# kunpengcompute/media

Measured on AMD Instinct MI355X. Metric: encoded fps @1080p I420 baseline-profile, 1/2/4/8 MI355X vs OpenH264 CPU, higher is better.
Workload: dtype u8

## Files before the change

### media_amd/csrc/engine.h

```cpp
#pragma once

#define HIPCHK(err, call)                                                                                    \
    do {                                                                                                     \
        hipError_t _r = (call);                                                                              \
        if (_r != hipSuccess) return set_err((err), MI355X_H264_E_HIP, "%s: %s", #call, hipGetErrorString(_r)); \
    } while (0)
namespace { thread_local const char* t_failed_call = ""; }
#define HIPTRY(call)                                                      \
    do {                                                                  \
        hipError_t _r = (call);                                           \
        if (_r != hipSuccess) { t_failed_call = #call; return _r; }       \
    } while (0)

namespace {

struct DevMem {
    struct Block { void* p; bool pinned; };
    std::vector<Block> blocks;
    template <class T> hipError_t dev(T** p, size_t bytes, bool zero = false)
    {
        HIPTRY(hipMalloc((void**)p, bytes));
        blocks.push_back({*p, false});
        if (zero) HIPTRY(hipMemset(*p, 0, bytes));
        return hipSuccess;
// ... 276 lines not shown
    }
    P.itemtab = T.d_itemtab; P.srctab = T.d_srctab; P.qtab = e->d_qtab; P.st_ring_y = e->st_ring_y; P.st_ring_c = e->st_ring_c; P.nbuf = e->nbuf;
    P.st_src = T.src_item_stride; P.sl = e->sl;
    P.band.row0 = e->b_row0; P.band.rows = e->b_rows;
    const unsigned pic_serial = P.pic_serial;
    const unsigned G = (unsigned)T.n;
    fill_qp(P.qy, P.qc, P.lambda, P.sad_nz, e->qp);
    P.search = e->cfg.search;
    const StepSync& Y = *T.sync;
    hipStream_t st = Y.st;


    if (T.inj) {
        const size_t n = (size_t)T.n * e->nmb;
        HIPCHK(e->err, hipMemcpyAsync(e->d_mb, T.inj->mbinfo, n * sizeof(MbInfo), hipMemcpyHostToDevice, st));
        HIPCHK(e->err, hipMemcpyAsync(e->d_levels, T.inj->levels, n * LV_STRIDE * sizeof(int16_t), hipMemcpyHostToDevice, st));
        HIPCHK(e->err, hipMemcpyAsync(e->d_mvq, T.inj->mvq, n * 8 * sizeof(int16_t), hipMemcpyHostToDevice, st));
        HIPCHK(e->err, hipMemcpyAsync(e->d_aux, T.inj->mbaux, n * 16, hipMemcpyHostToDevice, st));
        HIPCHK(e->err, hipMemsetAsync(e->d_me_cost, 0, n * sizeof(uint16_t), st));
        unsigned anypcm[MAX_BATCH] = {}, anyintra[MAX_BATCH] = {};
        const MbInfo* m = (const MbInfo*)T.inj->mbinfo;
        for (int g = 0; g < T.n; g++)
            for (int i = 0; i < e->nmb; i++) {
                const int type = m[(size_t)g * e->nmb + i].type;
                if (type == MB_IPCM) anypcm[g] = pic_serial;
                if (!idr && mb_is_intra_host(type)) anyintra[g] = pic_serial;
            }
        HIPCHK(e->err, hipMemcpyAsync(e->d_anypcm, anypcm, (size_t)T.n * sizeof(unsigned), hipMemcpyHostToDevice, st));
        HIPCHK(e->err, hipMemcpyAsync(e->d_anyintra, anyintra, (size_t)T.n * sizeof(unsigned), hipMemcpyHostToDevice, st));
        HIPCHK(e->err, hipStreamSynchronize(st));
    } else if (idr) {
        StatScope sc(e, &S, MI355X_H264_K_INTRA, (uint32_t)(e->diag_mode ? e->mbw + e->mbh - 1 : 1), (uint32_t)(e->b_nmb * T.n), st);
        LAUNCH2(ind, k_i4_decide<true>, k_i4_decide<false>, dim3((e->b_nmb + 3) / 4, G), dim3(64), st, P, 0);
        if (e->diag_mode && !ind) {
            for (int s = 0; s < e->mbw + e->mbh - 1; s++) {
                const int ymin = std::max(0, s - e->mbw + 1), ymax = std::min(e->mbh - 1, s);
                hipLaunchKernelGGL(k_intra_diag, dim3(ymax - ymin + 1, G), dim3(64), 0, st, P, s);
            }
        } else {
            const IntraRowParams R = intra_row_params(e, P, Y.h_err, (int)G);
            {
                static const int slots = getenv("MI355X_H264_INTRA_SLOTS") ? std::max(1, atoi(getenv("MI355X_H264_INTRA_SLOTS"))) : 24;
                LAUNCH2(ind, k_intra_rows<true>, k_intra_rows<false>, dim3(e->b_rows, std::min(G, (unsigned)slots)), dim3(128), st, R);
            }
        }
    } else {
        { const bool turns = g_turns_on && !ind && e->me_turn > 0 && T.n >= TURN_MIN_BATCH;
          if (turns) hipLaunchKernelGGL(k_turn_acquire, dim3(1), dim3(64), 0, st, g_turns.d_lock[e->device], (unsigned)e->me_turn, (int)TURN_TIMEOUT_US);
          { StatScope sc(e, &S, MI355X_H264_K_ME, (uint32_t)P.nref, (uint32_t)(e->b_nmb * T.n), st);
            FrameParams Q = P;
            Q.rf_last = P.nref - 1;
            for (int r = 0; r < P.nref; r++) {
                Q.rf = r;
                for (int p = 0; p < 3; p++) Q.ref[p] = P.refs[r][p];
                LAUNCH2(ind, k_me<true>, k_me<false>, dim3(e->b_nmb, G), dim3(64), st, Q);
            } }
          if (turns) hipLaunchKernelGGL(k_turn_release, dim3(1), dim3(1), 0, st, g_turns.d_lock[e->device], (unsigned)e->me_turn);
        }
        { StatScope sc(e, &S, MI355X_H264_K_PMB, 1, (uint32_t)(e->b_nmb * T.n), st);
          if (e->cfg.profile_idc == 100) LAUNCH2(ind, k_tq8<true>, k_tq8<false>, dim3((e->b_nmb + 15) / 16, G), dim3(64), st, P);
          else LAUNCH2(ind, k_tq<true>, k_tq<false>, dim3((e->b_nmb + 7) / 8, G), dim3(64), st, P); }
        {
            const IntraRowParams R = intra_row_params(e, P, Y.h_err, (int)G);
            static const int pslots_env = getenv("MI355X_H264_PINTRA_SLOTS") ? std::max(1, atoi(getenv("MI355X_H264_PINTRA_SLOTS"))) : 0;
            const unsigned pslots = std::min(G, pslots_env ? (unsigned)pslots_env : (e->p_intra_x16 > 16u * PINTRA_SPARSE_MBS ? G : 1u));
            LAUNCH2(ind, k_i4_decide<true>, k_i4_decide<false>, dim3(std::min((e->b_nmb + 3) / 4, (int)I4_MARKED_WAVES), pslots), dim3(64), st, P, (int)G);
            LAUNCH2(ind, (k_pintra_rows<false, true>), (k_pintra_rows<false, false>), dim3(e->b_rows, pslots), dim3(64), st, R);
        }
    }
    HdrBatch H{}, Hpcm{};
    for (int g = 0; g < T.n; g++) {
        uint64_t hdr = 0;
        const int fn = ind ? T.items[g].frame_num : e->seq.frame_num, qp = ind ? T.items[g].qp : e->qp;
        const int id = ind ? T.items[g].idr_id : ((e->seq.idr_id + g * e->idr_step) & 0xFF);
        const int nact = ind ? (idr ? 0 : 1) : avail_refs(e, idr);
        H.len[g] = (unsigned char)build_slice_header(e->shape, idr, id, false, fn, qp, nact, &hdr);
        H.bits[g] = hdr;
        Hpcm.len[g] = (unsigned char)build_slice_header(e->shape, idr, id, true, fn, qp, nact, &hdr);
        Hpcm.bits[g] = hdr;
    }
    hipStream_t ec = T.one_stream ? st : Y.ec;
    CavlcParams C{};
    C.mb = e->d_mb; C.levels = e->d_levels; C.mvd = e->d_mvd; C.mbw = e->mbw; C.nmb = e->nmb; C.p_slice = idr ? 0 : 1; C.t8x8 = e->cfg.profile_idc == 100 ? 1 : 0;
    C.nref = ind ? (idr ? 0 : 1) : avail_refs(e, idr); C.sl = e->sl;
    C.mb_first = e->b_row0 * e->mbw; C.mb_end = C.mb_first + e->b_nmb;
    C.slice_cap = (unsigned)e->slice_cap;
    C.mbdiv = P.mbdiv;
    C.slotbits = e->d_slotbits; C.slotcode = e->d_slotcode; C.mbbits = e->d_mbbits; C.bitbuf = S.d_bitbuf;
    C.bs = (uint8_t*)e->d_bs; C.prevcoded = e->d_prevcoded;
    C.st_mb = e->nmb; C.st_bitbuf = e->st_bitbuf_bytes / 4;
    C.aux = e->d_aux; C.mvq = e->d_mvq;
    C.src = T.d_src; C.w = e->cfg.width; C.h = e->cfg.height; C.src_nv12 = T.nv12 ? 1 : 0; C.st_src = T.src_item_stride;
    C.itemtab = T.d_itemtab; C.srctab = T.d_srctab;
    const int cavlc_grid = (e->b_nmb + 1) / 2;
    unsigned db_serial = 0;
    if (!e->cfg.disable_deblock) {
        db_serial = next_nonzero(e->serial);
        LAUNCH2(ind, k_bs<true>, k_bs<false>, dim3(std::min(cavlc_grid, (int)BS_WAVES), G), dim3(64), st, C, e->d_anybs, db_serial);
    }
    const bool fork = ec != st;
    if (fork) {
        HIPCHK(e->err, hipEventRecord(Y.recon_ready, st));
        HIPCHK(e->err, hipStreamWaitEvent(ec, Y.recon_ready, 0));
    }
    {
        StatScope sc(e, &S, MI355X_H264_K_CAVLC, 4, (uint32_t)(e->b_nmb * T.n), ec);
        const int grid = cavlc_grid;
        if (!idr) {
            LAUNCH2(ind, k_mvpred<true>, k_mvpred<false>, dim3((e->b_nmb + 63) / 64, G), dim3(64), ec, P);
            LAUNCH2(ind, k_skip_scan<true>, k_skip_scan<false>, dim3(G), dim3(256), ec, C);
        }
        LAUNCH2(ind, (k_cavlc<false, true>), (k_cavlc<false, false>), dim3(grid, G), dim3(64), ec, C);
        LAUNCH2(ind, k_bit_scan<true>, k_bit_scan<false>, dim3(G * (unsigned)e->b_nsl), dim3(SCAN_NT), ec, C, H, Hpcm, (const unsigned*)e->d_anypcm, pic_serial, S.d_info, e->d_me_cost,
                e->b_nsl, e->b_sl0, (unsigned)e->slice_cap);
        LAUNCH2(ind, (k_cavlc<true, true>), (k_cavlc<true, false>), dim3(grid, G), dim3(64), ec, C);
        const size_t pre = (idr ? e->sps_pps.size() : 0) + 5;
        const size_t pad = (16 - (pre & 15)) & 15;
        T.lay = AuLayout{pad, e->nsl > 1 ? 0 : pad + pre, idr, idr ? ((3 << 5) | 5) : ((2 << 5) | 1)};
        LAUNCH2(ind, k_pack<true>, k_pack<false>, dim3(G * (unsigned)e->b_nsl), dim3(SCAN_NT), ec, (uint8_t*)S.d_bitbuf, e->st_bitbuf_bytes, S.h_au + T.lay.payload_off, e->st_au,
                (const SliceInfo*)S.d_info, S.h_info, e->b_nsl, e->b_sl0, (unsigned)e->slice_cap, T.d_itemtab);
    }
    if (fork) HIPCHK(e->err, hipEventRecord(Y.entropy_done, ec));
    if (e->keep_pre && !ind && !T.inj)
        for (int p = 0; p < 3; p++) {
            const size_t ring = p ? e->st_ring_c : e->st_ring_y;
            HIPCHK(e->err, hipMemcpy2DAsync(e->d_pre[p], ring, e->d_planes[cur][p], p ? e->st_c : e->st_y, ring, (size_t)e->G, hipMemcpyDeviceToDevice, st));
        }
    if (e->keep_pre && ind)
        for (int k = 0; k < T.n; k++)
            for (int p = 0; p < 3; p++) {
                const size_t ring = p ? e->st_ring_c : e->st_ring_y;
                HIPCHK(e->err, hipMemcpyAsync(e->d_pre[p] + (size_t)T.items[k].item * ring,
                                              e->d_plane_base[p] + (size_t)T.items[k].item * (p ? e->st_c : e->st_y) + (size_t)T.items[k].cur * ring, ring,
                                              hipMemcpyDeviceToDevice, st));
            }
    if (!e->cfg.disable_deblock && !T.inj) {
        const int steps = e->mbw + 2 * (e->mbh - 1);
        StatScope sc(e, &S, MI355X_H264_K_DEBLOCK, (uint32_t)(e->diag_mode ? steps : 1), (uint32_t)(e->b_nmb * T.n), st);
        const DbParams D = db_params(e, ind ? e->d_plane_base : e->d_planes[cur], e->sl, e->qp);
        if (e->diag_mode && !ind) {
            for (int s = 0; s < steps; s++) {
                const int ymin = std::max(0, (s - (e->mbw - 1) + 1) >> 1), ymax = std::min(e->mbh - 1, s >> 1);
                if (ymax < ymin) continue;
                hipLaunchKernelGGL(k_deblock_diag, dim3(ymax - ymin + 1), dim3(64), 0, st, D, s);
            }
        } else {
            DbRowParams R = db_row_params(e, D, Y.h_err, db_serial, pic_serial, e->b_row0, (int)G);
            R.itemtab = T.d_itemtab; R.st_ring_y = e->st_ring_y; R.st_ring_c = e->st_ring_c;
            const bool pairs = e->pair_filter && T.n >= e->pair_min_batch && e->nsl == 1 && e->b_rows == e->mbh;
            const unsigned grid_x = pairs ? (unsigned)((e->b_rows + 1) / 2) : (unsigned)e->b_rows;
            auto filter = [&](bool bs4, unsigned at_a_time) {
                const dim3 grid(grid_x, std::min(G, at_a_time));
                if (pairs) { if (bs4) LAUNCH2(ind, (k_deblock_pairs<true, true>), (k_deblock_pairs<true, false>), grid, dim3(64), st, R);
                             else LAUNCH2(ind, (k_deblock_pairs<false, true>), (k_deblock_pairs<false, false>), grid, dim3(64), st, R); }
                else { if (bs4) LAUNCH2(ind, (k_deblock_rows<true, false, true>), (k_deblock_rows<true, false, false>), grid, dim3(64), st, R);
                       else LAUNCH2(ind, (k_deblock_rows<false, false, true>), (k_deblock_rows<false, false, false>), grid, dim3(64), st, R); }
            };
            if (idr) { R.need_intra = 0; filter(true, G); }
            else {
                R.need_intra = -1; filter(false, G);
                R.need_intra = 1; filter(true, e->p_intra_x16 > 16u * PINTRA_SPARSE_MBS ? G : 1u);
            }
        }
    }
    if (fork) HIPCHK(e->err, hipStreamWaitEvent(st, Y.entropy_done, 0));
    HIPCHK(e->err, hipEventRecord(Y.done, st));
    HIPCHK(e->err, hipGetLastError());
    return MI355X_H264_OK;
}

int submit(mi355x_h264_encoder* e, const uint8_t* d_src, size_t src_item_stride, int slot_idx, bool nv12, const Injected* inj = nullptr)
{
    Slot& S = e->slots[slot_idx];
    const bool idr = e->seq.next_is_idr(e->cfg.gop) || (e->after_injected && !inj);
    e->seq.begin(idr);
    e->after_injected = inj != nullptr;
    Step T;
    T.d_src = d_src; T.src_item_stride = src_item_stride; T.nv12 = nv12; T.idr = idr; T.n = e->G;
    T.sync = &S.sync;
    T.slot = &S;
    T.inj = inj;
    const int rc = submit_step(e, T);
    if (rc) return rc;
    S.lay = T.lay;
    S.busy = true;
    e->seq.advance(idr, e->nbuf, e->idr_step * e->G);
    return MI355X_H264_OK;
}

int wait_slot(mi355x_h264_encoder* e, int slot_idx)
{
    Slot& S = e->slots[slot_idx];
    if (!S.busy) return set_err(e->err, MI355X_H264_E_INTERNAL, "collect on an idle slot");
    HIPCHK(e->err, hipEventSynchronize(S.sync.done));
    S.busy = false;
    for (auto& ev : S.evs) {
        float ms = 0;
        if (hipEventElapsedTime(&ms, ev.a, ev.b) == hipSuccess) {
            e->stats.ms[ev.k] += ms; e->stats.launches[ev.k] += ev.launches; e->stats.mbs[ev.k] += ev.mbs;
        }
        e->ev_pool.push_back(ev.a); e->ev_pool.push_back(ev.b);
    }
    S.evs.clear();
    e->stats.frames += (uint64_t)e->G;
    const int rc = handoff_timeout(S.sync, e->err);
    if (rc) e->seq.force_idr = 1;
    return rc;
}

int finish_item(mi355x_h264_encoder* e, Slot& S, const AuLayout& L, int g, uint8_t** out, uint32_t* out_len, int* frame_type)
{
    uint8_t* base = S.h_au + (size_t)g * e->st_au;
    const SliceInfo* const info = S.h_info + (size_t)g * e->b_nsl;
    for (int sl = 0; sl < e->b_nsl; sl++)
        if (info[sl].error) {
            e->seq.force_idr = 1;
            const int code = info[sl].error == 1 ? MI355X_H264_E_OVERFLOW : MI355X_H264_E_INTERNAL;
            if (e->nsl > 1) return set_err(e->err, code, "device reported error %u (slice %d)", info[sl].error, sl);
            return set_err(e->err, code, "device reported error %u", info[sl].error);
        }
    uint32_t cost = 0, searched = 0, tq_coded = 0;
    size_t need = e->sps_pps.size() + 16;
    for (int sl = 0; sl < e->b_nsl; sl++) {
        cost += info[sl].me_cost; searched += info[sl].searched; tq_coded += info[sl].tq_coded;
        need += 5 + (size_t)info[sl].total_bytes * 3 / 2 + 16;
    }
    e->last_me_cost[g] = cost;
    if (!L.idr) {
        e->stats.p_mbs += (uint64_t)e->b_nmb; e->stats.me_searched_mbs += searched; e->stats.tq_coded_mbs += tq_coded;
        e->p_intra_x16 = (3 * e->p_intra_x16 + 16 * (searched - tq_coded)) / 4;
    }
    if (frame_type) *frame_type = L.idr ? MI355X_H264_FRAME_IDR : MI355X_H264_FRAME_P;
    std::vector<uint8_t>& eb = e->esc_buf[g];
    if (e->nsl > 1) {
        eb.resize(need);
        size_t pos = 0;
        if (L.idr && e->b_sl0 == 0) { memcpy(eb.data(), e->sps_pps.data(), e->sps_pps.size()); pos = e->sps_pps.size(); }
        for (int sl = 0; sl < e->b_nsl; sl++) {
            const SliceInfo& si = info[sl];
            const uint8_t* pay = base + (size_t)(e->b_sl0 + sl) * e->slice_cap;
            uint8_t* o = eb.data() + pos;
            o[0] = 0; o[1] = 0; o[2] = 0; o[3] = 1; o[4] = (uint8_t)L.nal_hdr;
            pos += 5;
            if (si.epb_count == 0) { memcpy(eb.data() + pos, pay, si.total_bytes); pos += si.total_bytes; }
            else pos += nal_escape(pay, si.total_bytes, eb.data() + pos);
        }
        *out = eb.data();
        *out_len = (uint32_t)pos;
        return MI355X_H264_OK;
    }
    uint8_t* au = base + L.au_start;
    size_t pos = 0;
    if (L.idr) { memcpy(au, e->sps_pps.data(), e->sps_pps.size()); pos = e->sps_pps.size(); }
    au[pos++] = 0; au[pos++] = 0; au[pos++] = 0; au[pos++] = 1; au[pos++] = (uint8_t)L.nal_hdr;
    if (info->epb_count == 0) {
        *out = au;
        *out_len = (uint32_t)(pos + info->total_bytes);
    } else {
        eb.resize(pos + (size_t)info->total_bytes * 3 / 2 + 16);
        memcpy(eb.data(), au, pos);
        const size_t n = nal_escape(base + L.payload_off, info->total_bytes, eb.data() + pos);
        *out = eb.data();
        *out_len = (uint32_t)(pos + n);
    }
    return MI355X_H264_OK;
}

int collect(mi355x_h264_encoder* e, int slot_idx, uint8_t** out, uint32_t* out_len, int* frame_type)
{
    const int rc = wait_slot(e, slot_idx);
    return rc ? rc : finish_item(e, e->slots[slot_idx], e->slots[slot_idx].lay, 0, out, out_len, frame_type);
}

void destroy_engine(mi355x_h264_encoder* e)
{
    if (!e) return;
    (void)hipSetDevice(e->device);
    if (e->stream) (void)hipStreamSynchronize(e->stream);
    if (e->stream_ec && e->stream_ec != e->stream) (void)hipStreamSynchronize(e->stream_ec);
    e->mem.free_all();
    for (auto& S : e->slots) {
        sync_destroy(S.sync);
        for (auto& ev : S.evs) { (void)hipEventDestroy(ev.a); (void)hipEventDestroy(ev.b); }
    }
    for (auto ev : e->ev_pool) (void)hipEventDestroy(ev);
    if (e->stream_ec && e->stream_ec != e->stream) (void)hipStreamDestroy(e->stream_ec);
    if (e->counted_live) e->counted_live->fetch_sub(1);
    if (e->stream) (void)hipStreamDestroy(e->stream);
    delete e;
}

hipError_t engine_alloc(mi355x_h264_encoder* e, bool hub_engine)
{
    DevMem& M = e->mem;
    HIPTRY(hipSetDevice(e->device));
    HIPTRY(hipStreamCreateWithFlags(&e->stream, hipStreamNonBlocking));
    {
        static std::atomic<int> live{0};
        const char* one = getenv("MI355X_H264_ONE_STREAM");
        const int n = live.fetch_add(1) + 1;
        e->counted_live = &live;
        if ((one && one[0] == '1') || (n > 2 && !(one && one[0] == '0'))) e->stream_ec = e->stream;
        else HIPTRY(hipStreamCreateWithFlags(&e->stream_ec, hipStreamNonBlocking));
    }
    const size_t ysz = (size_t)e->cw * e->ch;
    const size_t Gn = (size_t)e->G, nmb = Gn * e->nmb;
    e->st_ring_y = ysz + 256; e->st_ring_c = ysz / 4 + 256;
    e->st_y = e->st_ring_y * e->nbuf; e->st_c = e->st_ring_c * e->nbuf;
    for (int p = 0; p < 3; p++) {
        HIPTRY(M.dev(&e->d_plane_base[p], (p ? e->st_c : e->st_y) * Gn, true));
        for (int b = 0; b < e->nbuf; b++) e->d_planes[b][p] = e->d_plane_base[p] + (size_t)b * (p ? e->st_ring_c : e->st_ring_y);
    }
// ... 203 lines not shown
```

### media_amd/csrc/k_deblock.h

```cpp
#pragma once
#include "dev_common.h"

namespace h264 {

__constant__ const uint8_t c_alpha[52] = {0,  0,  0,  0,  0,  0,  0,  0,  0,  0,  0,  0,  0,   0,   0,   0,   4,   4,
                                          5,  6,  7,  8,  9,  10, 12, 13, 15, 17, 20, 22, 25,  28,  32,  36,  40,  45,
                                          50, 56, 63, 71, 80, 90, 101, 113, 127, 144, 162, 182, 203, 226, 255, 255};
__constant__ const uint8_t c_beta[52] = {0,  0,  0,  0,  0,  0,  0,  0,  0,  0,  0,  0,  0,  0,  0,  0,  2,  2,
                                         2,  3,  3,  3,  3,  4,  4,  4,  6,  6,  7,  7,  8,  8,  9,  9,  10, 10,
                                         11, 11, 12, 12, 13, 13, 14, 14, 15, 15, 16, 16, 17, 17, 18, 18};
__constant__ const uint8_t c_tc0[52][3] = {
    {0, 0, 0},   {0, 0, 0},   {0, 0, 0},    {0, 0, 0},    {0, 0, 0},    {0, 0, 0},   {0, 0, 0},   {0, 0, 0},  {0, 0, 0},
    {0, 0, 0},   {0, 0, 0},   {0, 0, 0},    {0, 0, 0},    {0, 0, 0},    {0, 0, 0},   {0, 0, 0},   {0, 0, 0},  {0, 0, 1},
    {0, 0, 1},   {0, 0, 1},   {0, 0, 1},    {0, 1, 1},    {0, 1, 1},    {1, 1, 1},   {1, 1, 1},   {1, 1, 1},  {1, 1, 1},
    {1, 1, 2},   {1, 1, 2},   {1, 1, 2},    {1, 1, 2},    {1, 2, 3},    {1, 2, 3},   {2, 2, 3},   {2, 2, 4},  {2, 3, 4},
    {2, 3, 4},   {3, 3, 5},   {3, 4, 6},    {3, 4, 6},    {4, 5, 7},    {4, 5, 8},   {4, 6, 9},   {5, 7, 10}, {6, 8, 11},
    {6, 8, 13},  {7, 10, 14}, {8, 11, 16},  {9, 12, 18},  {10, 13, 20}, {11, 15, 23}, {13, 17, 25}};

struct DbParams {
    uint8_t* pl[3];
    const MbInfo* mb;
    int cw, ch, mbw, mbh;
    int alpha_y, beta_y, alpha_c, beta_c;
    int tc0_y[3], tc0_c[3];
// ... 24 lines not shown
    const int ap = iabs(p2 - p0), aq = iabs(q2 - q0);
    if (bS < 4) {
        const int tc = tc0 + (ap < beta) + (aq < beta);
        const int d = clip3(-tc, tc, (((q0 - p0) << 2) + (p1 - q1) + 4) >> 3);
        pix[-xs] = (uint8_t)clip255(p0 + d);
        pix[0] = (uint8_t)clip255(q0 - d);
        if (ap < beta) pix[-2 * xs] = (uint8_t)(p1 + clip3(-tc0, tc0, (p2 + ((p0 + q0 + 1) >> 1) - (p1 << 1)) >> 1));
        if (aq < beta) pix[xs] = (uint8_t)(q1 + clip3(-tc0, tc0, (q2 + ((p0 + q0 + 1) >> 1) - (q1 << 1)) >> 1));
    } else {
        const int p3 = pix[-4 * xs], q3 = pix[3 * xs];
        const bool strong = iabs(p0 - q0) < ((alpha >> 2) + 2);
        if (ap < beta && strong) {
            pix[-xs] = (uint8_t)((p2 + 2 * p1 + 2 * p0 + 2 * q0 + q1 + 4) >> 3);
            pix[-2 * xs] = (uint8_t)((p2 + p1 + p0 + q0 + 2) >> 2);
            pix[-3 * xs] = (uint8_t)((2 * p3 + 3 * p2 + p1 + p0 + q0 + 4) >> 3);
        } else pix[-xs] = (uint8_t)((2 * p1 + p0 + q1 + 2) >> 2);
        if (aq < beta && strong) {
            pix[0] = (uint8_t)((p1 + 2 * p0 + 2 * q0 + 2 * q1 + q2 + 4) >> 3);
            pix[xs] = (uint8_t)((p0 + q0 + q1 + q2 + 2) >> 2);
            pix[2 * xs] = (uint8_t)((2 * q3 + 3 * q2 + q1 + q0 + p0 + 4) >> 3);
        } else pix[0] = (uint8_t)((2 * q1 + q0 + p1 + 2) >> 2);
    }
}

enum { DB_LP = 24, DB_CP = 12 };

__global__ __launch_bounds__(64) void k_deblock_diag(DbParams D, int s)
{
    const int lane = threadIdx.x;
    const int ymin = max(0, (s - (D.mbw - 1) + 1) >> 1);
    const int my = ymin + blockIdx.x, mx = s - 2 * my;
    if (my >= D.mbh || mx < 0 || mx >= D.mbw) return;
    const int cs = D.cw / 2;
    __shared__ __attribute__((aligned(16))) uint8_t s_y[20 * DB_LP];
    __shared__ __attribute__((aligned(16))) uint8_t s_c[2][10 * DB_CP];
    __shared__ uint8_t s_bs[2][16];

    for (int i = lane; i < 20 * 5; i += 64) {
        const int r = i / 5, c = i - r * 5;
        const int gy = 16 * my - 4 + r, gx = 16 * mx - 4 + c * 4;
        uint32_t v = 0;
        if (gy >= 0 && gx >= 0) v = *(const uint32_t*)(D.pl[0] + (size_t)gy * D.cw + gx);
        *(uint32_t*)(s_y + r * DB_LP + c * 4) = v;
    }
    for (int i = lane; i < 2 * 10 * 5; i += 64) {
        const int pl = i / 50, k = i - pl * 50, r = k / 5, c = k - r * 5;
        const int gy = 8 * my - 2 + r, gx = 8 * mx - 2 + c * 2;
        uint16_t v = 0;
        if (gy >= 0 && gx >= 0) v = *(const uint16_t*)(D.pl[1 + pl] + (size_t)gy * cs + gx);
        *(uint16_t*)(s_c[pl] + r * DB_CP + c * 2) = v;
    }
    if (lane < 32) {
        const int dir = lane >> 4, e = (lane >> 2) & 3, k = lane & 3;
        const int bS = D.bs[((size_t)my * D.mbw + mx) * 32 + lane];
        s_bs[dir][e * 4 + k] = (uint8_t)bS;
    }
    __syncthreads();

    const bool isY = lane < 16, isC = lane >= 16 && lane < 32;
    const int cpl = (lane >> 3) & 1, cl = lane & 7;
#pragma unroll 1
    for (int dir = 0; dir < 2; dir++) {
#pragma unroll 1
        for (int e = 0; e < 4; e++) {
            if (isY) {
                const int bS = s_bs[dir][e * 4 + (lane >> 2)];
                if (bS) {
                    uint8_t* p = dir == 0 ? s_y + (4 + lane) * DB_LP + 4 + 4 * e : s_y + (4 + 4 * e) * DB_LP + 4 + lane;
                    filter_line(p, dir == 0 ? 1 : DB_LP, bS, D.alpha_y, D.beta_y, bS < 4 ? D.tc0_y[bS - 1] : 0, false);
                }
            } else if (isC && !(e & 1)) {
                const int bS = s_bs[dir][e * 4 + (cl >> 1)];
                if (bS) {
                    uint8_t* p = dir == 0 ? s_c[cpl] + (2 + cl) * DB_CP + 2 + 2 * e : s_c[cpl] + (2 + 2 * e) * DB_CP + 2 + cl;
                    filter_line(p, dir == 0 ? 1 : DB_CP, bS, D.alpha_c, D.beta_c, bS < 4 ? D.tc0_c[bS - 1] : 0, true);
                }
            }
            __syncthreads();
        }
    }
    for (int i = lane; i < 20 * 5; i += 64) {
        const int r = i / 5, c = i - r * 5;
        const int gy = 16 * my - 4 + r, gx = 16 * mx - 4 + c * 4;
        if (gy < 0 || gx < 0) continue;
        if (r < 4 && c == 0) continue;
        *(uint32_t*)(D.pl[0] + (size_t)gy * D.cw + gx) = *(const uint32_t*)(s_y + r * DB_LP + c * 4);
    }
    for (int i = lane; i < 2 * 10 * 5; i += 64) {
        const int pl = i / 50, k = i - pl * 50, r = k / 5, c = k - r * 5;
        const int gy = 8 * my - 2 + r, gx = 8 * mx - 2 + c * 2;
        if (gy < 0 || gx < 0) continue;
        if (r < 2 && c == 0) continue;
        *(uint16_t*)(D.pl[1 + pl] + (size_t)gy * cs + gx) = *(const uint16_t*)(s_c[pl] + r * DB_CP + c * 2);
    }
}

typedef unsigned long long u64;
#define AT_LOAD(p) __hip_atomic_load((p), __ATOMIC_RELAXED, __HIP_MEMORY_SCOPE_AGENT)
#define AT_STORE(p, v) __hip_atomic_store((p), (v), __ATOMIC_RELAXED, __HIP_MEMORY_SCOPE_AGENT)

struct DbRowParams {
    DbParams d;
    u64* handoff;
    const uint32_t* bs;
    unsigned* err;
    unsigned serial;
    const unsigned* anybs;
    const unsigned* anypcm;
    const unsigned* anyintra;
    unsigned pic_serial;
    int npic;
    int need_intra;
    size_t st_y, st_c, st_handoff;
    int st_mb;
    int row0;
    const uint32_t* itemtab;
    size_t st_ring_y, st_ring_c;
    const DecPos* dectab;
};

template <bool BS4>
__device__ __forceinline__ void filt_uni(const int p3, int& p2, int& p1, int& p0, int& q0, int& q1, int& q2, const int q3,
                                         int bS, bool chroma, int alpha, int beta, int t1, int t2, int t3)
{
    const int tc0 = bS == 1 ? t1 : (bS == 2 ? t2 : t3);
    const int fm = -(int)(bS != 0 && iabs(p0 - q0) < alpha && iabs(p1 - p0) < beta && iabs(q1 - q0) < beta);
    const int lum = chroma ? 0 : -1;
    const int apm = lum & -(int)(iabs(p2 - p0) < beta), aqm = lum & -(int)(iabs(q2 - q0) < beta);
    const int tc = tc0 + (chroma ? 1 : 0) - apm - aqm;
    const int d = clip3(-tc, tc, (((q0 - p0) << 2) + (p1 - q1) + 4) >> 3);
    const int avg = (p0 + q0 + 1) >> 1;
    int dp0 = clip255(p0 + d) - p0, dq0 = clip255(q0 - d) - q0;
    int dp1 = apm & clip3(-tc0, tc0, (p2 + avg - (p1 << 1)) >> 1);
    int dq1 = aqm & clip3(-tc0, tc0, (q2 + avg - (q1 << 1)) >> 1);
    int dp2 = 0, dq2 = 0;
    if (BS4) {
        const int s4 = -(int)(bS == 4);
        const int strong = -(int)(iabs(p0 - q0) < ((alpha >> 2) + 2));
        const int sp = apm & strong, sq = aqm & strong;
        const int wp0 = (sp & (((p2 + 2 * p1 + 2 * p0 + 2 * q0 + q1 + 4) >> 3) - p0)) | (~sp & (((2 * p1 + p0 + q1 + 2) >> 2) - p0));
        const int wq0 = (sq & (((p1 + 2 * p0 + 2 * q0 + 2 * q1 + q2 + 4) >> 3) - q0)) | (~sq & (((2 * q1 + q0 + p1 + 2) >> 2) - q0));
        const int wp1 = sp & (((p2 + p1 + p0 + q0 + 2) >> 2) - p1), wq1 = sq & (((p0 + q0 + q1 + q2 + 2) >> 2) - q1);
        const int wp2 = sp & (((2 * p3 + 3 * p2 + p1 + p0 + q0 + 4) >> 3) - p2), wq2 = sq & (((2 * q3 + 3 * q2 + q1 + q0 + p0 + 4) >> 3) - q2);
        dp0 = (s4 & wp0) | (~s4 & dp0); dq0 = (s4 & wq0) | (~s4 & dq0);
        dp1 = (s4 & wp1) | (~s4 & dp1); dq1 = (s4 & wq1) | (~s4 & dq1);
        dp2 = s4 & wp2; dq2 = s4 & wq2;
    }
    p0 += fm & dp0; q0 += fm & dq0; p1 += fm & dp1; q1 += fm & dq1;
    if (BS4) { p2 += fm & dp2; q2 += fm & dq2; }
}

enum { DR_LP = 40, DR_CP = 24 };
enum { DR_CB = 4 * 201, DR_CPS = 4 * 144, DR_TILE = DR_CB + 2 * DR_CPS + 12 };
__device__ __forceinline__ uint8_t* db_y(uint8_t* const tile, const int r, const int c) { return tile + (r + 4) * DR_LP + c + 16; }
__device__ __forceinline__ uint8_t* db_c(uint8_t* const tile, const int pl, const int r, const int c) { return tile + DR_CB + pl * DR_CPS + (r + 4) * DR_CP + c + 8; }
__device__ __forceinline__ uint32_t& dw(uint8_t* const p) { return *(uint32_t*)p; }

struct DbThr { int al, be, t1, t2, t3; };
__device__ __forceinline__ DbThr db_picture_thr(const DbParams& D, const bool isC)
{
    return isC ? DbThr{D.alpha_c, D.beta_c, D.tc0_c[0], D.tc0_c[1], D.tc0_c[2]} : DbThr{D.alpha_y, D.beta_y, D.tc0_y[0], D.tc0_y[1], D.tc0_y[2]};
}
template <bool PERMB, bool IND>
__device__ __forceinline__ bool db_picture_view(const DbRowParams& R, const int pos, DbParams& D, u64*& handoff, const uint32_t*& bsw)
{
    if constexpr (PERMB) {
        const DecPosRef dp = dec_pos(R.dectab, pos);
        if (!dp.filtered || R.anybs[dp.item] != R.serial) return false;
        if (R.need_intra != 0 && dp.intra != (R.need_intra > 0)) return false;
        D = R.d;
        const size_t g = (size_t)dp.item;
        D.pl[0] += g * R.st_y + (size_t)dp.cur * R.st_ring_y; D.pl[1] += g * R.st_c + (size_t)dp.cur * R.st_ring_c; D.pl[2] += g * R.st_c + (size_t)dp.cur * R.st_ring_c;
        D.mb += g * R.st_mb; D.mbqp += g * R.st_mb;
        D.oa = dp.oa; D.ob = dp.ob; D.cqo_cb = dp.cqo_cb; D.cqo_cr = dp.cqo_cr; D.sl = dp.fsl;
        handoff = R.handoff + g * R.st_handoff;
        bsw = R.bs + g * R.st_mb * 8;
        return true;
    } else {
    const int bitem = batch_item<IND>(R.itemtab, pos);
    if (R.anybs[bitem] != R.serial) return false;
    if (R.anypcm[bitem] == R.pic_serial) return false;
    if (R.need_intra != 0 && (R.anyintra[bitem] == R.pic_serial) != (R.need_intra > 0)) return false;
    D = R.d;
    const size_t g = (size_t)bitem;
    D.pl[0] += g * R.st_y; D.pl[1] += g * R.st_c; D.pl[2] += g * R.st_c; D.mb += g * R.st_mb;
    if constexpr (IND) {
        const ItemRef it = item_ref(R.itemtab, pos);
        D.pl[0] += (size_t)it.cur * R.st_ring_y; D.pl[1] += (size_t)it.cur * R.st_ring_c; D.pl[2] += (size_t)it.cur * R.st_ring_c;
        const int qpc = c_chroma_qp[it.qp];
        D.alpha_y = c_alpha[it.qp]; D.beta_y = c_beta[it.qp]; D.alpha_c = c_alpha[qpc]; D.beta_c = c_beta[qpc];
#pragma unroll
        for (int i = 0; i < 3; i++) { D.tc0_y[i] = c_tc0[it.qp][i]; D.tc0_c[i] = c_tc0[qpc][i]; }
    }
    handoff = R.handoff + g * R.st_handoff;
    bsw = R.bs + g * R.st_mb * 8;
    return true;
    }
}
struct DbLane { bool isC; int fpl, seg8, hstride; uint8_t *vrow, *hcol; };
__device__ __forceinline__ DbLane db_lane(const int l, uint8_t* const tile)
{
    DbLane L;
    L.isC = l >= 16; L.fpl = (l >> 3) & 1;
    const int fln = L.isC ? (l & 7) : l;
    L.seg8 = 8 * (L.isC ? (fln >> 1) : (fln >> 2));
    L.vrow = L.isC ? db_c(tile, L.fpl, fln, -4) : db_y(tile, fln, -4);
    L.hcol = L.isC ? db_c(tile, L.fpl, -4, fln) : db_y(tile, -4, fln);
    L.hstride = L.isC ? DR_CP : DR_LP;
    return L;
}
template <bool BS4, int E>
__device__ __forceinline__ bool db_edge(const DbLane& L, int (&px)[20], const uint4 b, const DbThr& T)
{
    const uint32_t w = E == 0 ? b.x : E == 1 ? (L.isC ? b.z : b.y) : E == 2 ? b.z : b.w;
    const int bS = (E >= 2 && L.isC) ? 0 : (int)((w >> L.seg8) & 255);
    if (__ballot(bS != 0) == 0ull) return false;
    filt_uni<BS4>(px[4 * E], px[4 * E + 1], px[4 * E + 2], px[4 * E + 3], px[4 * E + 4], px[4 * E + 5], px[4 * E + 6], px[4 * E + 7],
                  bS, L.isC, T.al, T.be, T.t1, T.t2, T.t3);
    return true;
}
template <int W>
__device__ __forceinline__ uint32_t db_pack(const int (&px)[20])
{
    return (uint32_t)px[4 * W] | ((uint32_t)px[4 * W + 1] << 8) | ((uint32_t)px[4 * W + 2] << 16) | ((uint32_t)px[4 * W + 3] << 24);
}
template <bool BS4>
__device__ __forceinline__ void db_left_edge(const DbLane& L, int (&px)[20], const uint4 b0, const bool on, const DbThr& T)
{
    if (on) {
#pragma unroll
        for (int w = 0; w < 5; w++) {
            const uint32_t v = dw(L.vrow + 4 * w);
#pragma unroll
            for (int b = 0; b < 4; b++) px[4 * w + b] = (int)((v >> (8 * b)) & 255);
        }
        if (db_edge<BS4, 0>(L, px, b0, T)) dw(L.vrow) = db_pack<0>(px);
    }
}
template <bool BS4>
__device__ __forceinline__ void db_inner_vertical(const DbLane& L, int (&px)[20], const uint4 b0, const bool on, const DbThr& T)
{
    if (on) {
        db_edge<BS4, 1>(L, px, b0, T);
        db_edge<BS4, 2>(L, px, b0, T);
        db_edge<BS4, 3>(L, px, b0, T);
        dw(L.vrow + 4) = db_pack<1>(px); dw(L.vrow + 8) = db_pack<2>(px);
        if (!L.isC) { dw(L.vrow + 12) = db_pack<3>(px); dw(L.vrow + 16) = db_pack<4>(px); }
    }
}
template <bool BS4>
__device__ __forceinline__ void db_horizontal(const DbLane& L, const uint4 b1, const bool on, const DbThr& Ttop, const DbThr& T)
{
    if (on) {
        int px[20];
#pragma unroll
        for (int r = 0; r < 20; r++) px[r] = L.hcol[r * L.hstride];
        db_edge<BS4, 0>(L, px, b1, Ttop);
        db_edge<BS4, 1>(L, px, b1, T);
        db_edge<BS4, 2>(L, px, b1, T);
        db_edge<BS4, 3>(L, px, b1, T);
#pragma unroll
        for (int r = 1; r < 19; r++) {
            const bool both = r == 3 || r == 4 || r == 7 || r == 8;
            if (both || !L.isC) L.hcol[r * L.hstride] = (uint8_t)px[r];
        }
    }
}
template <class F>
__device__ __forceinline__ void db_granule(const int k, F f)
{
    if (k < 16) f(false, 0, 12 + (k >> 2), (k & 3) * 4);
    else if (k < 24) f(true, (k - 16) >> 2, 6 + (((k - 16) >> 1) & 1), ((k - 16) & 1) * 4);
}
__device__ __forceinline__ uint8_t* db_tile_at(uint8_t* const tile, const bool c, const int pl, const int r, const int col, const int dmx, const int dmy)
{
    return c ? db_c(tile, pl, 8 * dmy + r, 8 * dmx + col) : db_y(tile, 16 * dmy + r, 16 * dmx + col);
}
__device__ __forceinline__ uint32_t db_bottom_dword(uint8_t* const tile, const int k, const bool shifted)
{
    uint32_t v = 0;
    db_granule(k, [&](bool c, int pl, int r, int col) { v = dw(db_tile_at(tile, c, pl, r, col, shifted ? -1 : 0, 0)); });
    return v;
}
__device__ __forceinline__ void db_put_apron(uint8_t* const tile, const int k, const uint32_t v)
{
    db_granule(k, [&](bool c, int pl, int r, int col) { dw(db_tile_at(tile, c, pl, r, col, 0, -1)) = v; });
}
__device__ __forceinline__ void db_store_apron(const DbParams& D, uint8_t* const tile, const int k, const int mx, const int my)
{
    db_granule(k, [&](bool c, int pl, int r, int col) {
        uint8_t* const p = c ? (pl ? D.pl[2] : D.pl[1]) + (size_t)(8 * (my - 1) + r) * (D.cw / 2) + 8 * mx + col
                             : D.pl[0] + (size_t)(16 * (my - 1) + r) * D.cw + 16 * mx + col;
        dw(p) = dw(db_tile_at(tile, c, pl, r, col, 0, -1));
    });
}
__device__ __forceinline__ void db_wait_tags(const bool need, u64& g, const u64* const addr, const unsigned serial, bool& timed_out)
{
    unsigned spins = 0;
    while (!timed_out) {
        const bool bad = need && (unsigned)(g >> 32) != serial;
        if (__ballot(bad) == 0ull) break;
        if (++spins > (1u << 20)) { timed_out = true; break; }
        __builtin_amdgcn_s_sleep(1);
        if (need) g = AT_LOAD(addr);
    }
}

template <bool BS4, bool PERMB, bool IND>
__device__ __forceinline__ void deblock_rows_picture(const DbRowParams& R, const int pos)
{
    DbParams D; u64* handoff; const uint32_t* bsw;
    if (!db_picture_view<PERMB, IND>(R, pos, D, handoff, bsw)) return;
    const int lane = threadIdx.x, my = R.row0 + blockIdx.x, cs = D.cw / 2;
    const bool first_row = !D.sl.has_top(my);
    const bool last_row = my == D.mbh - 1 || !D.sl.has_top(my + 1);
    __shared__ __attribute__((aligned(16))) uint8_t s_y[DR_TILE];
    bool timed_out = false;
    const int yr = lane >> 2, yc4 = (lane & 3) * 4;
    const int cpl_l = (lane >> 4) & 1, cr_l = (lane >> 1) & 7, cc4 = (lane & 1) * 4;
    const DbLane L = db_lane(lane, s_y);
    DbThr thr = db_picture_thr(D, L.isC), thrL = thr, thrT = thr;
    __shared__ uint32_t s_tA[PERMB ? 52 : 1];
    __shared__ uint8_t s_tB[PERMB ? 52 : 1], s_cq[PERMB ? 52 : 1];
    if (PERMB) {
        if (lane < 52) {
            s_tA[lane] = ((uint32_t)c_alpha[lane] << 24) | ((uint32_t)c_tc0[lane][2] << 16) | ((uint32_t)c_tc0[lane][1] << 8) | (uint32_t)c_tc0[lane][0];
            s_tB[lane] = c_beta[lane];
            s_cq[lane] = c_chroma_qp[lane];
        }
        wave_sync();
    }
    const int cqo = L.fpl ? D.cqo_cr : D.cqo_cb;
    auto thresholds = [&](const int qa, const int qb) {
        const int ca = (int)s_cq[clip3(0, 51, qa + cqo)], cb = (int)s_cq[clip3(0, 51, qb + cqo)];
        const int av = ((L.isC ? ca : qa) + (L.isC ? cb : qb) + 1) >> 1;
        const uint32_t w = s_tA[clip3(0, 51, av + D.oa)];
        return DbThr{(int)(w >> 24), (int)s_tB[clip3(0, 51, av + D.ob)], (int)(w & 255u), (int)((w >> 8) & 255u), (int)((w >> 16) & 255u)};
    };
    uint32_t pf_q = 0;
    int qp_left = 0;

    uint32_t pf_y = 0, pf_c = 0;
    uint4 pf_b0 = {0, 0, 0, 0}, pf_b1 = pf_b0;
    u64 pf_g = 0;
    const int grow = first_row ? my : my - 1;
    const int glane = lane < 24 ? lane : lane - 24 < 24 ? lane - 24 : lane - 48;
    auto prefetch = [&](int mx) {
        pf_y = *(const uint32_t*)(D.pl[0] + (size_t)(16 * my + yr) * D.cw + 16 * mx + yc4);
        pf_c = *(const uint32_t*)((cpl_l ? D.pl[2] : D.pl[1]) + (size_t)(8 * my + cr_l) * cs + 8 * mx + cc4);
        const uint4* b = (const uint4*)(bsw + ((size_t)my * D.mbw + mx) * 8);
        pf_b0 = b[0]; pf_b1 = b[1];
        pf_g = AT_LOAD(handoff + ((size_t)grow * D.mbw + mx) * 24 + glane);
        if (PERMB) pf_q = (uint32_t)D.mbqp[(size_t)my * D.mbw + mx] | ((uint32_t)D.mbqp[(size_t)grow * D.mbw + mx] << 8);
    };
    auto consume = [&]() {
        asm volatile("" : "+v"(pf_y), "+v"(pf_c), "+v"(pf_g));
        asm volatile("" : "+v"(pf_b0.x), "+v"(pf_b0.y), "+v"(pf_b0.z), "+v"(pf_b0.w));
        asm volatile("" : "+v"(pf_b1.x), "+v"(pf_b1.y), "+v"(pf_b1.z), "+v"(pf_b1.w));
        if (PERMB) asm volatile("" : "+v"(pf_q));
    };
    prefetch(0);
    consume();
    uint32_t cur_y = pf_y, cur_c = pf_c, cur_q = pf_q;
    uint4 b0 = pf_b0, b1 = pf_b1;
    u64 g = pf_g;

    auto store_prev = [&](const int mx, const bool have_cur) {
        if (mx > 0) {
            const int pmx = mx - 1;
            const int co = have_cur ? -16 : 0, cco = have_cur ? -8 : 0;
            const int nrow = last_row ? 16 : 12, ncrow = last_row ? 8 : 6;
            if (yr < nrow) *(uint32_t*)(D.pl[0] + (size_t)(16 * my + yr) * D.cw + 16 * pmx + yc4) = dw(db_y(s_y, yr, co + yc4));
            if (lane < 32 && cr_l < ncrow)
                *(uint32_t*)((cpl_l ? D.pl[2] : D.pl[1]) + (size_t)(8 * my + cr_l) * cs + 8 * pmx + cc4) = dw(db_c(s_y, cpl_l, cr_l, cco + cc4));
            if (!last_row && lane < 24)
                AT_STORE(handoff + ((size_t)my * D.mbw + pmx) * 24 + lane, ((u64)R.serial << 32) | db_bottom_dword(s_y, lane, have_cur));
        }
    };
    for (int mx = 0; mx <= D.mbw; mx++) {
        const bool have_cur = mx < D.mbw;
        if (have_cur) {
            if (mx > 0) {
                dw(db_y(s_y, yr, yc4 - 16)) = dw(db_y(s_y, yr, yc4));
                if (lane < 32) dw(db_c(s_y, cpl_l, cr_l, cc4 - 8)) = dw(db_c(s_y, cpl_l, cr_l, cc4));
            }
            wave_sync();
            dw(db_y(s_y, yr, yc4)) = cur_y;
            if (lane < 32) dw(db_c(s_y, cpl_l, cr_l, cc4)) = cur_c;
            if (mx + 1 < D.mbw) prefetch(mx + 1);
            if (PERMB) {
                const int qc = (int)(cur_q & 255u), qt = (int)(cur_q >> 8);
                thr = thresholds(qc, qc);
                thrL = thresholds(mx > 0 ? qp_left : qc, qc);
                thrT = thresholds(qt, qc);
                qp_left = qc;
            }
            wave_sync();
            const bool v_on = (b0.x | b0.y | b0.z | b0.w) != 0 && lane < 32, h_on = (b1.x | b1.y | b1.z | b1.w) != 0 && lane < 32;
            int px[20];
            db_left_edge<BS4>(L, px, b0, v_on, thrL);
            wave_sync();
            store_prev(mx, true);
            db_inner_vertical<BS4>(L, px, b0, v_on, thr);
            if (!first_row) {
                db_wait_tags(lane < 24, g, handoff + ((size_t)grow * D.mbw + mx) * 24 + glane, R.serial, timed_out);
                db_put_apron(s_y, lane, (uint32_t)g);
            }
            wave_sync();
            db_horizontal<BS4>(L, b1, h_on, thrT, thr);
            wave_sync();
            consume();
            if (!first_row) db_store_apron(D, s_y, lane, mx, my);
        }
        if (!have_cur) store_prev(mx, false);
        cur_y = pf_y; cur_c = pf_c; b0 = pf_b0; b1 = pf_b1; g = pf_g; cur_q = pf_q;
        wave_sync();
    }
    if (timed_out && lane == 0) *R.err = 1u;
}
template <bool BS4, bool PERMB = false, bool IND = false>
__global__ __launch_bounds__(64) void k_deblock_rows(DbRowParams R)
{
    static_assert(!PERMB || IND, "thresholds per edge: the pictures of a decoder group's step");
    __builtin_amdgcn_s_setprio(3);
    for (int pos = blockIdx.y; pos < R.npic; pos += gridDim.y) deblock_rows_picture<BS4, PERMB, IND>(R, pos);
}


template <bool BS4, bool IND>
__device__ __forceinline__ void deblock_pairs_picture(const DbRowParams& R, const int pos)
{
    DbParams D; u64* handoff; const uint32_t* bsw;
    if (!db_picture_view<false, IND>(R, pos, D, handoff, bsw)) return;
    const int lane = threadIdx.x, half = lane >> 5, hl = lane & 31, cs = D.cw / 2;
    const int rowA = R.row0 + 2 * (int)blockIdx.x, rowB = rowA + 1;
    const bool hasB = rowB < D.mbh;
    const int my = half ? (hasB ? rowB : rowA) : rowA;
    const bool live = half == 0 || hasB;
    const bool first_row = half == 0 && rowA == 0;
    const bool last_row = my == D.mbh - 1;
    const bool from_lds = half == 1;
    __shared__ __attribute__((aligned(16))) uint8_t s_yy[2][(DR_TILE + 127) / 128 * 128];
    __shared__ __attribute__((aligned(16))) uint32_t s_ring[2][24];
    uint8_t* const s_y = s_yy[half];
    bool timed_out = false;
    const int yr0 = hl >> 2, yc4 = (hl & 3) * 4;
    const int cpl_l = (hl >> 4) & 1, cr_l = (hl >> 1) & 7, cc4 = (hl & 1) * 4;
    const DbLane L = db_lane(hl, s_y);
    const DbThr thr = db_picture_thr(D, L.isC);

    uint32_t pf_y0 = 0, pf_y1 = 0, pf_c = 0;
    uint4 pf_b0 = {0, 0, 0, 0}, pf_b1 = pf_b0;
    u64 pf_g = 0;
    const int grow = (first_row || half == 1) ? rowA : rowA - 1;
    const int glane = hl < 24 ? hl : hl - 24;
    const int last_mx = D.mbw - 1;
    auto prefetch = [&](int mx) {
        pf_y0 = *(const uint32_t*)(D.pl[0] + (size_t)(16 * my + yr0) * D.cw + 16 * mx + yc4);
        pf_y1 = *(const uint32_t*)(D.pl[0] + (size_t)(16 * my + yr0 + 8) * D.cw + 16 * mx + yc4);
        pf_c = *(const uint32_t*)((cpl_l ? D.pl[2] : D.pl[1]) + (size_t)(8 * my + cr_l) * cs + 8 * mx + cc4);
        const uint4* b = (const uint4*)(bsw + ((size_t)my * D.mbw + mx) * 8);
        pf_b0 = b[0]; pf_b1 = b[1];
        pf_g = AT_LOAD(handoff + ((size_t)grow * D.mbw + mx) * 24 + glane);
    };
    auto consume = [&]() {
        asm volatile("" : "+v"(pf_y0), "+v"(pf_y1), "+v"(pf_c), "+v"(pf_g));
        asm volatile("" : "+v"(pf_b0.x), "+v"(pf_b0.y), "+v"(pf_b0.z), "+v"(pf_b0.w));
        asm volatile("" : "+v"(pf_b1.x), "+v"(pf_b1.y), "+v"(pf_b1.z), "+v"(pf_b1.w));
    };
    prefetch(0);
    consume();
    uint32_t cur_y0 = pf_y0, cur_y1 = pf_y1, cur_c = pf_c;
    uint4 b0 = pf_b0, b1 = pf_b1;
    u64 g = pf_g;

    auto store_prev = [&](const int mx, const bool have_cur) {
        if (mx > 0 && live) {
            const int pmx = mx - 1;
            const int co = have_cur ? -16 : 0, cco = have_cur ? -8 : 0;
            const int nrow = last_row ? 16 : 12, ncrow = last_row ? 8 : 6;
            *(uint32_t*)(D.pl[0] + (size_t)(16 * my + yr0) * D.cw + 16 * pmx + yc4) = dw(db_y(s_y, yr0, co + yc4));
            if (yr0 + 8 < nrow) *(uint32_t*)(D.pl[0] + (size_t)(16 * my + yr0 + 8) * D.cw + 16 * pmx + yc4) = dw(db_y(s_y, yr0 + 8, co + yc4));
            if (cr_l < ncrow)
                *(uint32_t*)((cpl_l ? D.pl[2] : D.pl[1]) + (size_t)(8 * my + cr_l) * cs + 8 * pmx + cc4) = dw(db_c(s_y, cpl_l, cr_l, cco + cc4));
            if (!last_row && hl < 24) {
                const uint32_t v = db_bottom_dword(s_y, hl, have_cur);
                if (half == 0) s_ring[pmx & 1][hl] = v;
                else AT_STORE(handoff + ((size_t)my * D.mbw + pmx) * 24 + hl, ((u64)R.serial << 32) | v);
            }
        }
    };
    for (int t = 0; t <= D.mbw + 1; t++) {
        const int mx = t - half;
        const bool in_range = mx >= 0 && mx <= D.mbw && live;
        const bool have_cur = in_range && mx < D.mbw;
        if (have_cur) {
            if (mx > 0) {
                dw(db_y(s_y, yr0, yc4 - 16)) = dw(db_y(s_y, yr0, yc4));
                dw(db_y(s_y, yr0 + 8, yc4 - 16)) = dw(db_y(s_y, yr0 + 8, yc4));
                dw(db_c(s_y, cpl_l, cr_l, cc4 - 8)) = dw(db_c(s_y, cpl_l, cr_l, cc4));
            }
        }
        wave_sync();
        if (have_cur) {
            dw(db_y(s_y, yr0, yc4)) = cur_y0;
            dw(db_y(s_y, yr0 + 8, yc4)) = cur_y1;
            dw(db_c(s_y, cpl_l, cr_l, cc4)) = cur_c;
        }
        {
            const int nx = mx + 1 < 0 ? 0 : (mx + 1 > last_mx ? last_mx : mx + 1);
            prefetch(nx);
        }
        wave_sync();
        const bool v_on = have_cur && (b0.x | b0.y | b0.z | b0.w) != 0, h_on = have_cur && (b1.x | b1.y | b1.z | b1.w) != 0;
        int px[20];
        db_left_edge<BS4>(L, px, b0, v_on, thr);
        wave_sync();
        if (in_range) store_prev(mx, have_cur);
        db_inner_vertical<BS4>(L, px, b0, v_on, thr);
        wave_sync();
        db_wait_tags(have_cur && !from_lds && !first_row && hl < 24, g, handoff + ((size_t)grow * D.mbw + mx) * 24 + glane, R.serial, timed_out);
        if (have_cur && !first_row && hl < 24) db_put_apron(s_y, hl, from_lds ? s_ring[mx & 1][hl] : (uint32_t)g);
        wave_sync();
        db_horizontal<BS4>(L, b1, h_on, thr, thr);
        wave_sync();
        consume();
        if (have_cur && !first_row && hl < 24) db_store_apron(D, s_y, hl, mx, my);
        if (mx + 1 >= 0 && mx + 1 <= last_mx) { cur_y0 = pf_y0; cur_y1 = pf_y1; cur_c = pf_c; b0 = pf_b0; b1 = pf_b1; g = pf_g; }
        wave_sync();
    }
    if (timed_out && lane == 0) *R.err = 1u;
}
template <bool BS4, bool IND = false>
__global__ __launch_bounds__(64) void k_deblock_pairs(DbRowParams R)
{
    __builtin_amdgcn_s_setprio(3);
    for (int pos = blockIdx.y; pos < R.npic; pos += gridDim.y) deblock_pairs_picture<BS4, IND>(R, pos);
}

}
```

Before: 27530.

## Fuse P-frame deblock passes into one launch choosing BS4 variant per picture

For non-independent P frames, the two deblock launches (a non-intra pass, then an intra pass) are replaced by one kernel. It checks a per-picture any-intra flag and runs either the BS4 or the non-BS4 row/pair filter, so each picture is walked once. Shared-memory tiles move to kernel scope so both template instantiations share them. A ballot-gated re-request of stale handoff tags is added early in each step to cut time spent waiting on neighbour rows. Register pressure and code size may rise because both variants now sit in one kernel.

```diff
diff --git a/media_amd/csrc/engine.h b/media_amd/csrc/engine.h
--- a/media_amd/csrc/engine.h
+++ b/media_amd/csrc/engine.h
@@ -452,12 +452,16 @@
             auto filter = [&](bool bs4, unsigned at_a_time) {
                 const dim3 grid(grid_x, std::min(G, at_a_time));
                 if (pairs) { if (bs4) LAUNCH2(ind, (k_deblock_pairs<true, true>), (k_deblock_pairs<true, false>), grid, dim3(64), st, R);
-                             else LAUNCH2(ind, (k_deblock_pairs<false, true>), (k_deblock_pairs<false, false>), grid, dim3(64), st, R); }
+                             else hipLaunchKernelGGL((k_deblock_pairs<false, true>), grid, dim3(64), 0, st, R); }
                 else { if (bs4) LAUNCH2(ind, (k_deblock_rows<true, false, true>), (k_deblock_rows<true, false, false>), grid, dim3(64), st, R);
-                       else LAUNCH2(ind, (k_deblock_rows<false, false, true>), (k_deblock_rows<false, false, false>), grid, dim3(64), st, R); }
+                       else hipLaunchKernelGGL((k_deblock_rows<false, false, true>), grid, dim3(64), 0, st, R); }
             };
             if (idr) { R.need_intra = 0; filter(true, G); }
-            else {
+            else if (!ind) {
+                R.need_intra = 0;
+                if (pairs) hipLaunchKernelGGL(k_deblock_pairs_p, dim3(grid_x, G), dim3(64), 0, st, R);
+                else hipLaunchKernelGGL(k_deblock_rows_p, dim3(grid_x, G), dim3(64), 0, st, R);
+            } else {
                 R.need_intra = -1; filter(false, G);
                 R.need_intra = 1; filter(true, e->p_intra_x16 > 16u * PINTRA_SPARSE_MBS ? G : 1u);
             }
diff --git a/media_amd/csrc/k_deblock.h b/media_amd/csrc/k_deblock.h
--- a/media_amd/csrc/k_deblock.h
+++ b/media_amd/csrc/k_deblock.h
@@ -200,6 +200,7 @@
 
 enum { DR_LP = 40, DR_CP = 24 };
 enum { DR_CB = 4 * 201, DR_CPS = 4 * 144, DR_TILE = DR_CB + 2 * DR_CPS + 12 };
+enum { DR_PAIR_TILE = (DR_TILE + 127) / 128 * 128 };
 __device__ __forceinline__ uint8_t* db_y(uint8_t* const tile, const int r, const int c) { return tile + (r + 4) * DR_LP + c + 16; }
 __device__ __forceinline__ uint8_t* db_c(uint8_t* const tile, const int pl, const int r, const int c) { return tile + DR_CB + pl * DR_CPS + (r + 4) * DR_CP + c + 8; }
 __device__ __forceinline__ uint32_t& dw(uint8_t* const p) { return *(uint32_t*)p; }
@@ -353,16 +354,23 @@
         if (need) g = AT_LOAD(addr);
     }
 }
+__device__ __forceinline__ void db_rerequest(const bool need, u64& g, const u64* const addr, const unsigned serial)
+{
+    const bool bad = need && (unsigned)(g >> 32) != serial;
+    if (__ballot(bad) != 0ull) {
+        if (bad) g = AT_LOAD(addr);
+        asm volatile("" ::: "memory");
+    }
+}
 
 template <bool BS4, bool PERMB, bool IND>
-__device__ __forceinline__ void deblock_rows_picture(const DbRowParams& R, const int pos)
+__device__ __forceinline__ void deblock_rows_picture(const DbRowParams& R, const int pos, const int lane, uint8_t* const s_y)
 {
     DbParams D; u64* handoff; const uint32_t* bsw;
     if (!db_picture_view<PERMB, IND>(R, pos, D, handoff, bsw)) return;
-    const int lane = threadIdx.x, my = R.row0 + blockIdx.x, cs = D.cw / 2;
+    const int my = R.row0 + blockIdx.x, cs = D.cw / 2;
     const bool first_row = !D.sl.has_top(my);
     const bool last_row = my == D.mbh - 1 || !D.sl.has_top(my + 1);
-    __shared__ __attribute__((aligned(16))) uint8_t s_y[DR_TILE];
     bool timed_out = false;
     const int yr = lane >> 2, yc4 = (lane & 3) * 4;
     const int cpl_l = (lane >> 4) & 1, cr_l = (lane >> 1) & 7, cc4 = (lane & 1) * 4;
@@ -435,6 +443,7 @@
             wave_sync();
             dw(db_y(s_y, yr, yc4)) = cur_y;
             if (lane < 32) dw(db_c(s_y, cpl_l, cr_l, cc4)) = cur_c;
+            if (!first_row) db_rerequest(lane < 24, g, handoff + ((size_t)grow * D.mbw + mx) * 24 + glane, R.serial);
             if (mx + 1 < D.mbw) prefetch(mx + 1);
             if (PERMB) {
                 const int qc = (int)(cur_q & 255u), qt = (int)(cur_q >> 8);
@@ -470,17 +479,33 @@
 __global__ __launch_bounds__(64) void k_deblock_rows(DbRowParams R)
 {
     static_assert(!PERMB || IND, "thresholds per edge: the pictures of a decoder group's step");
+    __shared__ __attribute__((aligned(16))) uint8_t s_y[DR_TILE];
     __builtin_amdgcn_s_setprio(3);
-    for (int pos = blockIdx.y; pos < R.npic; pos += gridDim.y) deblock_rows_picture<BS4, PERMB, IND>(R, pos);
+    for (int pos = blockIdx.y; pos < R.npic; pos += gridDim.y) deblock_rows_picture<BS4, PERMB, IND>(R, pos, (int)threadIdx.x, s_y);
+}
+__device__ __forceinline__ bool db_picture_has_intra(const DbRowParams& R, const int pos)
+{
+    return R.anyintra[batch_item<false>(R.itemtab, pos)] == R.pic_serial;
+}
+__global__ __launch_bounds__(64) void k_deblock_rows_p(DbRowParams R)
+{
+    __shared__ __attribute__((aligned(16))) uint8_t s_y[DR_TILE];
+    __builtin_amdgcn_s_setprio(3);
+    for (int pos = blockIdx.y; pos < R.npic; pos += gridDim.y) {
+        int lane = threadIdx.x;
+        asm volatile("" : "+v"(lane));
+        if (db_picture_has_intra(R, pos)) deblock_rows_picture<true, false, false>(R, pos, lane, s_y);
+        else deblock_rows_picture<false, false, false>(R, pos, lane, s_y);
+    }
 }
 
 
 template <bool BS4, bool IND>
-__device__ __forceinline__ void deblock_pairs_picture(const DbRowParams& R, const int pos)
+__device__ __forceinline__ void deblock_pairs_picture(const DbRowParams& R, const int pos, const int lane, uint8_t (* const s_yy)[DR_PAIR_TILE], uint32_t (* const s_ring)[24])
 {
     DbParams D; u64* handoff; const uint32_t* bsw;
     if (!db_picture_view<false, IND>(R, pos, D, handoff, bsw)) return;
-    const int lane = threadIdx.x, half = lane >> 5, hl = lane & 31, cs = D.cw / 2;
+    const int half = lane >> 5, hl = lane & 31, cs = D.cw / 2;
     const int rowA = R.row0 + 2 * (int)blockIdx.x, rowB = rowA + 1;
     const bool hasB = rowB < D.mbh;
     const int my = half ? (hasB ? rowB : rowA) : rowA;
@@ -488,8 +513,6 @@
     const bool first_row = half == 0 && rowA == 0;
     const bool last_row = my == D.mbh - 1;
     const bool from_lds = half == 1;
-    __shared__ __attribute__((aligned(16))) uint8_t s_yy[2][(DR_TILE + 127) / 128 * 128];
-    __shared__ __attribute__((aligned(16))) uint32_t s_ring[2][24];
     uint8_t* const s_y = s_yy[half];
     bool timed_out = false;
     const int yr0 = hl >> 2, yc4 = (hl & 3) * 4;
@@ -555,6 +578,7 @@
             dw(db_y(s_y, yr0 + 8, yc4)) = cur_y1;
             dw(db_c(s_y, cpl_l, cr_l, cc4)) = cur_c;
         }
+        db_rerequest(have_cur && !from_lds && !first_row && hl < 24, g, handoff + ((size_t)grow * D.mbw + mx) * 24 + glane, R.serial);
         {
             const int nx = mx + 1 < 0 ? 0 : (mx + 1 > last_mx ? last_mx : mx + 1);
             prefetch(nx);
@@ -582,8 +606,22 @@
 template <bool BS4, bool IND = false>
 __global__ __launch_bounds__(64) void k_deblock_pairs(DbRowParams R)
 {
+    __shared__ __attribute__((aligned(16))) uint8_t s_yy[2][DR_PAIR_TILE];
+    __shared__ __attribute__((aligned(16))) uint32_t s_ring[2][24];
     __builtin_amdgcn_s_setprio(3);
-    for (int pos = blockIdx.y; pos < R.npic; pos += gridDim.y) deblock_pairs_picture<BS4, IND>(R, pos);
-}
-
-}
+    for (int pos = blockIdx.y; pos < R.npic; pos += gridDim.y) deblock_pairs_picture<BS4, IND>(R, pos, (int)threadIdx.x, s_yy, s_ring);
+}
+__global__ __launch_bounds__(64) void k_deblock_pairs_p(DbRowParams R)
+{
+    __shared__ __attribute__((aligned(16))) uint8_t s_yy[2][DR_PAIR_TILE];
+    __shared__ __attribute__((aligned(16))) uint32_t s_ring[2][24];
+    __builtin_amdgcn_s_setprio(3);
+    for (int pos = blockIdx.y; pos < R.npic; pos += gridDim.y) {
+        int lane = threadIdx.x;
+        asm volatile("" : "+v"(lane));
+        if (db_picture_has_intra(R, pos)) deblock_pairs_picture<true, false>(R, pos, lane, s_yy, s_ring);
+        else deblock_pairs_picture<false, false>(R, pos, lane, s_yy, s_ring);
+    }
+}
+
+}
```

After: 27920, median of 6. 1.4% higher.
